# ZechengLi19/CIM

Measured on AMD Instinct MI355X. Metric: images/sec training step (ResNet-50 VOC, ~1k proposals/img) at 1/2/4/8 GPU, higher is better.
Workload: dtype fp32

## Files before the change

cim_amd/csrc/gemm_pair.hip:

```cpp
#include "common.h"
#include <type_traits>
#include "../../include/cim_hip.h"

namespace {

using f32x16 = __attribute__((ext_vector_type(16))) float;
using f16x8 = __attribute__((ext_vector_type(8))) _Float16;
typedef short s16x4 __attribute__((__vector_size__(4 * sizeof(short))));
typedef short s16x8 __attribute__((__vector_size__(8 * sizeof(short))));

#ifndef CIM_PAIR_EXP
#define CIM_PAIR_EXP 0
#endif
static_assert(CIM_PAIR_EXP == 0 || (CIM_PAIR_EXP >= 3 && CIM_PAIR_EXP <= 5), "CIM_PAIR_EXP: 0 (product), 3, 4 or 5");
constexpr bool ABL_NO_LOOP_DMA = CIM_PAIR_EXP == 3 || CIM_PAIR_EXP == 5;
constexpr bool ABL_NO_LOOP_READS = CIM_PAIR_EXP == 4 || CIM_PAIR_EXP == 5;

constexpr int BM = 256, BN = 256, BK = 32;
constexpr int NW = 8, NT = 64 * NW;
constexpr int WNC = 4;
constexpr int WM = 128, WN = BN / WNC, MI = 4, NI = WN / 32;
constexpr int IPW = 32 / NW;
constexpr int OPER = 256 * BK * 4;
constexpr int SLAB = 2 * OPER;
constexpr int LDS_BYTES = 2 * SLAB;
constexpr int RBM = 128, RBK = 16, RNT = 256, RSTAGES = 5;
constexpr int RSTAGE_A = RBM * RBK * 4, RSTAGE_B = BN * RBK * 4, RSTAGE = RSTAGE_A + RSTAGE_B;
constexpr int RIPA = RSTAGE_A / 1024 / 4, RIPB = RSTAGE_B / 1024 / 4;
constexpr int RLDS_BYTES = RSTAGES * RSTAGE;

enum { L_KC = 0, L_MC = 1 };

struct PairArgs {
    const char* A;
    const char* B;
    float* C;
    const float* bias;
    int M, N, K;
    int lda, ldb, ldc;
    int relu;
    int k_per_split;
    long long c_split_stride;
    int batch;
    long long a_bs, b_bs, c_bs;
    const float* a_scale;
    const float* b_scale;
    unsigned* c_amax;
    int tn, tm, tz;
    int tile0;
};

typedef __attribute__((address_space(3))) char* lds_ptr_t;

__device__ __forceinline__ void glds16x4(const char* sbase, unsigned o0, unsigned o1, unsigned o2, unsigned o3, unsigned lds_dst) {
    unsigned keep;
    asm volatile(
        "s_mov_b32 %0, m0\n\t"
        "s_mov_b32 m0, %6\n\t"
        "s_nop 4\n\t"
        "global_load_lds_dwordx4 %1, %5\n\t"
        "s_addk_i32 m0, 0x400\n\t"
        "s_nop 0\n\t"
        "global_load_lds_dwordx4 %2, %5\n\t"
        "s_addk_i32 m0, 0x400\n\t"
        "s_nop 0\n\t"
        "global_load_lds_dwordx4 %3, %5\n\t"
        "s_addk_i32 m0, 0x400\n\t"
        "s_nop 0\n\t"
        "global_load_lds_dwordx4 %4, %5\n\t"
        "s_mov_b32 m0, %0"
        : "=&s"(keep)
// ... 153 lines not shown
__device__ __forceinline__ unsigned abs_bits(float x) { return __float_as_uint(x) & 0x7fffffffu; }
__device__ __forceinline__ unsigned abs_bits(unsigned x) { return x & 0x7fffffffu; }
template <class V4>
__device__ __forceinline__ unsigned abs_bits_max4(const V4& v) {
    return max(max(abs_bits(v.x), abs_bits(v.y)), max(abs_bits(v.z), abs_bits(v.w)));
}

__device__ __forceinline__ void block_amax_publish(unsigned* word, unsigned v) {
    __shared__ unsigned s_m[4];
    v = wave_max_u32(v);
    if ((threadIdx.x & 63) == 0) s_m[threadIdx.x >> 6] = v;
    __syncthreads();
    if (threadIdx.x == 0) cim::amax_publish(word, max(max(s_m[0], s_m[1]), max(s_m[2], s_m[3])));
}

template <int TBM, int SLABK>
struct PairTile {
    int tile_m, tile_n, m0, n0;
    const char* A;
    const char* B;
    float* C;
    int zsplit, zb;
    int kbeg, nslab;
    __device__ __forceinline__ explicit PairTile(const PairArgs& g) {
        int zidx;
        pair_tile_map(g.M, g.N, g.tn, g.tm, g.tz, (int)blockIdx.x + g.tile0, tile_m, tile_n, zidx);
        m0 = tile_m * TBM;
        n0 = tile_n * BN;
        A = g.A;
        B = g.B;
        C = g.C;
        zsplit = zidx;
        zb = 0;
        if (g.batch > 1) {
            A += (size_t)zidx * g.a_bs * 4;
            B += (size_t)zidx * g.b_bs * 4;
            C += (size_t)zidx * g.c_bs;
            zsplit = 0;
            zb = zidx;
        }
        kbeg = zsplit * g.k_per_split;
        const int kend = min(g.K, kbeg + g.k_per_split);
        nslab = (kend - kbeg) / SLABK;
    }
};

__device__ __forceinline__ void pair_acc_init(const PairArgs& g, int ncol0, int lane, f32x16 (&acc)[MI][NI], float (&bvj)[NI]) {
#pragma unroll
    for (int i = 0; i < MI; ++i)
#pragma unroll
        for (int j = 0; j < NI; ++j)
#pragma unroll
            for (int r = 0; r < 16; ++r) acc[i][j][r] = 0.0f;
#pragma unroll
    for (int j = 0; j < NI; ++j) {
        const int n = ncol0 + j * 32 + (lane & 31);
        bvj[j] = (g.bias != nullptr && n < g.N) ? g.bias[n] : 0.0f;
    }
}

template <class Loop>
__device__ __forceinline__ void for_valid_subtiles(int rows, Loop&& loop) {
    switch (__builtin_amdgcn_readfirstlane(min(MI, (rows + 31) / 32))) {
        case 1: loop(std::integral_constant<int, 1>{}); break;
        case 2: loop(std::integral_constant<int, 2>{}); break;
        case 3: loop(std::integral_constant<int, 3>{}); break;
        default: loop(std::integral_constant<int, MI>{}); break;
    }
}

template <int MIV>
struct PairFrags {
    f16x8 ah[MIV > 0 ? MIV : 1], al[MIV > 0 ? MIV : 1], bh[NI], bl[NI];
};

template <int MIV>
__device__ __forceinline__ void mma_cluster(f32x16 (&acc)[MI][NI], const f16x8 (&af)[MIV], const f16x8 (&bf)[NI]) {
#pragma unroll
    for (int i = 0; i < MIV; ++i)
#pragma unroll
        for (int j = 0; j < NI; ++j) acc[i][j] = __builtin_amdgcn_mfma_f32_32x32x16_f16(af[i], bf[j], acc[i][j], 0, 0, 0);
}

template <int NMFMA, int NREAD>
__device__ __forceinline__ void interleave_mfma_reads() {
#pragma unroll
    for (int q = 0; q < NMFMA; ++q) {
        __builtin_amdgcn_sched_group_barrier(0x008, 1, 0);
        if (q < NREAD) __builtin_amdgcn_sched_group_barrier(0x100, 1, 0);
    }
    if constexpr (NREAD > NMFMA) __builtin_amdgcn_sched_group_barrier(0x100, NREAD - NMFMA, 0);
    __builtin_amdgcn_sched_barrier(0);
}

template <int TBM, int SLABK>
__device__ __forceinline__ void pair_epilogue(const PairArgs& g, const PairTile<TBM, SLABK>& T, f32x16 (&acc)[MI][NI], float (&bvj)[NI],
                                              int wm, int wn, int lane) {
    const float inv = 1.0f / (g.a_scale[T.zb] * g.b_scale[T.zb]);
#pragma unroll
    for (int j = 0; j < NI; ++j) asm volatile("" : "+v"(bvj[j]));
    float* C = T.C + (size_t)T.zsplit * g.c_split_stride;
    const int m0 = T.m0, n0 = T.n0;
    const int lk = lane >> 5, l31 = lane & 31;
    unsigned amax = 0;
    const bool relu = g.relu != 0;
    if (m0 + TBM <= g.M && n0 + BN <= g.N) {
#pragma unroll
        for (int j = 0; j < NI; ++j) {
            float* cj = C + (size_t)(m0 + wm * WM + 4 * lk) * g.ldc + n0 + wn * WN + j * 32 + l31;
#pragma unroll
            for (int i = 0; i < MI; ++i) {
#pragma unroll
                for (int r = 0; r < 16; ++r) {
                    float v = acc[i][j][r] * inv + bvj[j];
                    if (relu) v = fmaxf(v, 0.0f);
                    amax = max(amax, abs_bits(v));
                    cj[(size_t)(i * 32 + (r & 3) + 8 * (r >> 2)) * g.ldc] = v;
                }
            }
        }
    } else {
#pragma unroll
        for (int j = 0; j < NI; ++j) {
            const int n = n0 + wn * WN + j * 32 + l31;
            if (n >= g.N) continue;
#pragma unroll
            for (int i = 0; i < MI; ++i) {
#pragma unroll
                for (int r = 0; r < 16; ++r) {
                    const int m = m0 + wm * WM + i * 32 + (r & 3) + 8 * (r >> 2) + 4 * lk;
                    if (m >= g.M) continue;
                    float v = acc[i][j][r] * inv + bvj[j];
                    if (relu) v = fmaxf(v, 0.0f);
                    amax = max(amax, abs_bits(v));
                    C[(size_t)m * g.ldc + n] = v;
                }
            }
        }
    }
    if (g.c_amax != nullptr && g.c_split_stride == 0) {
        amax = wave_max_u32(amax);
        if (lane == 0) cim::amax_publish(g.c_amax, amax);
    }
}

template <int AL, int BL, bool ONEP>
__global__ __launch_bounds__(NT, NW / 4) void gemm_pair_kernel(const PairArgs g) {
    extern __shared__ __attribute__((aligned(16))) char smem[];
    const int tid = threadIdx.x;
    const int wave = __builtin_amdgcn_readfirstlane(tid >> 6), lane = tid & 63;
    const int wm = wave / WNC, wn = wave % WNC;
    const PairTile<BM, BK> T(g);
    const int nslab = T.nslab;

    using StageA = typename StageSel<AL, BM, IPW>::type;
    using StageB = typename StageSel<BL, BN, IPW>::type;
    StageA sa;
    StageB sb;
    sa.init(T.m0, g.M, g.lda, wave, lane);
    sb.init(T.n0, g.N, g.ldb, wave, lane);
    const char* ak = T.A + (AL == L_KC ? (size_t)T.kbeg * 4 : (size_t)T.kbeg * g.lda * 4);
    const char* bk = T.B + (BL == L_KC ? (size_t)T.kbeg * 4 : (size_t)T.kbeg * g.ldb * 4);
    const size_t a_adv = StageA::k_step_bytes(g.lda), b_adv = StageB::k_step_bytes(g.ldb);

    typename FragSel<AL, MI, BM>::type fa;
    typename FragSel<BL, NI, BN>::type fb;
    fa.init(wm * WM, lane);
    fb.init(wn * WN, lane);

    f32x16 acc[MI][NI];
    float bvj[NI];
    pair_acc_init(g, T.n0 + wn * WN, lane, acc, bvj);

    auto issue_slab = [&](const char* buf, auto with_a) __attribute__((always_inline)) {
        if constexpr (decltype(with_a)::value) sa.issue(ak, buf, wave);
        sb.issue(bk, buf + OPER, wave);
        ak += a_adv;
        bk += b_adv;
    };
    auto prologue = [&](auto with_a) __attribute__((always_inline)) {
        issue_slab(smem, with_a);
        asm volatile("s_waitcnt vmcnt(0)" ::: "memory");
        __syncthreads();
        if (nslab > 1) issue_slab(smem + SLAB, with_a);
    };
    auto slab_loop = [&](auto miv_c) {
        constexpr int MIV = decltype(miv_c)::value;
        constexpr std::bool_constant<(MIV > 0 || AL == L_MC)> with_a{};
        PairFrags<MIV> f0, f1;
        auto read = [&](PairFrags<MIV>& f, const char* buf, int ks, auto in_loop) __attribute__((always_inline)) {
            if constexpr (MIV == 0) {
            } else if constexpr (ABL_NO_LOOP_READS && decltype(in_loop)::value) {
                asm volatile("" : "+v"(f.ah[0]), "+v"(f.al[0]), "+v"(f.bh[0]), "+v"(f.bl[0]));
            } else {
#pragma unroll
// ... 50 lines not shown
template <bool ONEP>
__global__ __launch_bounds__(RNT, 2) void gemm_pair_ring_kernel(const PairArgs g) {
    extern __shared__ __attribute__((aligned(16))) char smem[];
    const int tid = threadIdx.x;
    const int wave = __builtin_amdgcn_readfirstlane(tid >> 6), lane = tid & 63;
    const int wn = wave;
    const PairTile<RBM, RBK> T(g);
    const int nslab = T.nslab;

    const char* ak = T.A + (size_t)T.kbeg * g.lda * 4;
    const char* bk = T.B + (size_t)T.kbeg * g.ldb * 4;
    const size_t a_adv = (size_t)RBK * g.lda * 4, b_adv = (size_t)RBK * g.ldb * 4;
    StageMC<RBM, RIPA, RBK> sa;
    StageMC<BN, RIPB, RBK> sb;
    sa.init(T.m0, g.M, g.lda, wave, lane);
    sb.init(T.n0, g.N, g.ldb, wave, lane);
    FragMC<MI, RBM> fa;
    FragMC<NI, BN> fb;
    fa.init(0, lane);
    fb.init(wn * WN, lane);

    f32x16 acc[MI][NI];
    float bvj[NI];
    pair_acc_init(g, T.n0 + wn * WN, lane, acc, bvj);

    int left = nslab - 1;
    auto advance = [&]() __attribute__((always_inline)) {
        const bool more = left > 0;
        ak += more ? a_adv : 0;
        bk += more ? b_adv : 0;
        left -= more ? 1 : 0;
    };
#pragma unroll
    for (int q = 0; q < RSTAGES - 1; ++q) {
        sa.issue(ak, smem + q * RSTAGE, wave);
        sb.issue(bk, smem + q * RSTAGE + RSTAGE_A, wave);
        advance();
    }
    asm volatile("s_waitcnt vmcnt(18)" ::: "memory");
    __syncthreads();

    auto main_loop = [&](auto miv_c) {
        constexpr int MIV = decltype(miv_c)::value;
        PairFrags<MIV> f0, f1;
        auto read_b = [&](PairFrags<MIV>& f, const char* buf) __attribute__((always_inline)) {
#pragma unroll
            for (int j = 0; j < NI; ++j) {
// ... 33 lines not shown
                read_a(nf.ah, nxt, 0);
                mma_cluster(acc, f.ah, f.bh);
                interleave_mfma_reads<MIV * NI, 2 * MIV>();
                sb.issue_pair(bk, wbuf + RSTAGE_A, wave, 1);
            }
            advance();
            wb = wb == RSTAGES - 1 ? 0 : wb + 1;
            rb = rb == RSTAGES - 1 ? 0 : rb + 1;
        };
        read_b(f0, smem);
        if constexpr (!ONEP) read_a(f0.al, smem, 1);
        read_a(f0.ah, smem, 0);
        for (int t = 0; t < nslab; t += 2) {
            step(f0, f1);
            step(f1, f0);
        }
    };
    for_valid_subtiles(g.M - T.m0, main_loop);
    asm volatile("s_waitcnt vmcnt(0)" ::: "memory");
    pair_epilogue(g, T, acc, bvj, 0, wn, lane);
}

__global__ __launch_bounds__(256) void pair_splitk_reduce_kernel(const float* __restrict__ ws, float* __restrict__ C,
                                                                 const float* __restrict__ bias, int M, int N, int ldc,
                                                                 int splits, long long stride, int relu,
                                                                 unsigned* __restrict__ c_amax) {
    const long long total = (long long)M * N;
    unsigned am = 0;
    for (long long i = ((long long)blockIdx.x * 256 + threadIdx.x) * 4; i < total; i += (long long)gridDim.x * 1024) {
        const int m = (int)(i / N), n = (int)(i % N);
        float4 s = *reinterpret_cast<const float4*>(ws + i);
        for (int k0 = 1; k0 < splits; k0 += 4) {
            float4 v[4];
#pragma unroll
            for (int j = 0; j < 4; ++j)
                v[j] = k0 + j < splits ? *reinterpret_cast<const float4*>(ws + (long long)(k0 + j) * stride + i) : make_float4(0.f, 0.f, 0.f, 0.f);
#pragma unroll
            for (int j = 0; j < 4; ++j)
                if (k0 + j < splits) { s.x += v[j].x; s.y += v[j].y; s.z += v[j].z; s.w += v[j].w; }
        }
        if (bias) {
            const float4 b = *reinterpret_cast<const float4*>(bias + n);
            s.x += b.x; s.y += b.y; s.z += b.z; s.w += b.w;
        }
        if (relu) {
            s.x = fmaxf(s.x, 0.f); s.y = fmaxf(s.y, 0.f); s.z = fmaxf(s.z, 0.f); s.w = fmaxf(s.w, 0.f);
        }
        *reinterpret_cast<float4*>(C + (size_t)m * ldc + n) = s;
        am = max(am, abs_bits_max4(s));
    }
    if (c_amax != nullptr) block_amax_publish(c_amax, am);
}

using cim::pair_split2;
using cim::pair_scale_of;

__global__ __launch_bounds__(256) void pair_masked_stats_kernel(const float* __restrict__ dy, const float* __restrict__ y, int rows,
                                                                int cols, float* __restrict__ part, unsigned* __restrict__ amax) {
    __shared__ float4 red[16][16];
// ... 58 lines not shown
            a = make_float4(ya.x > 0.f ? a.x : 0.f, ya.y > 0.f ? a.y : 0.f, ya.z > 0.f ? a.z : 0.f, ya.w > 0.f ? a.w : 0.f);
            b = make_float4(yb.x > 0.f ? b.x : 0.f, yb.y > 0.f ? b.y : 0.f, yb.z > 0.f ? b.z : 0.f, yb.w > 0.f ? b.w : 0.f);
        }
        pair_split2(a.x * s, a.y * s, h.x, l.x);
        pair_split2(a.z * s, a.w * s, h.y, l.y);
        pair_split2(b.x * s, b.y * s, h.z, l.z);
        pair_split2(b.z * s, b.w * s, h.w, l.w);
    }
    char* dst = P + ((size_t)z * p_bs + (size_t)r * ldp + c * 8) * 4;
    *reinterpret_cast<uint4*>(dst) = h;
    *reinterpret_cast<uint4*>(dst + 16) = l;
}

__global__ __launch_bounds__(256) void pair_amax_kernel(const float* __restrict__ X, long long n4, int tail, unsigned* __restrict__ out) {
    unsigned m = 0;
    if (blockIdx.x == 0 && (int)threadIdx.x < tail) m = abs_bits(X[n4 * 4 + threadIdx.x]);
    for (long long i = (long long)blockIdx.x * 256 + threadIdx.x; i < n4; i += (long long)gridDim.x * 256) {
        const uint4 v = *reinterpret_cast<const uint4*>(X + i * 4);
        m = max(m, abs_bits_max4(v));
    }
    block_amax_publish(out, m);
}

template <int AL, int BL, bool RING>
int launch_pair(PairArgs g, int splits, float* workspace, hipStream_t st, int max_workgroups, int products) {
    static_assert(!RING || (AL == L_MC && BL == L_MC), "the ring kernel is the weight gradients' layout only");
    constexpr int TBM = RING ? RBM : BM, LDSB = RING ? RLDS_BYTES : LDS_BYTES, THREADS = RING ? RNT : NT;
    const int tm = (g.M + TBM - 1) / TBM, tn = (g.N + BN - 1) / BN;
    void (*kern)(const PairArgs);
    if constexpr (RING) kern = products == 1 ? gemm_pair_ring_kernel<true> : gemm_pair_ring_kernel<false>;
    else kern = products == 1 ? gemm_pair_kernel<AL, BL, true> : gemm_pair_kernel<AL, BL, false>;
    hipError_t e = hipFuncSetAttribute(reinterpret_cast<const void*>(kern), hipFuncAttributeMaxDynamicSharedMemorySize, LDSB);
    if (e != hipSuccess) return (int)e;
    const int slabs = g.K / BK;
    if (splits < 1) splits = 1;
    if (splits > slabs) splits = slabs;
    g.k_per_split = ((slabs + splits - 1) / splits) * BK;
    splits = (g.K + g.k_per_split - 1) / g.k_per_split;
    float* out = g.C;
    const float* bias = g.bias;
    const int relu = g.relu, ldc = g.ldc;
    if (splits > 1) {
        if (g.batch > 1) return -1;
        g.C = workspace;
        g.ldc = g.N;
        g.c_split_stride = (long long)g.M * g.N;
        g.bias = nullptr;
        g.relu = 0;
    } else {
        g.c_split_stride = 0;
    }
    g.tn = tn; g.tm = tm; g.tz = g.batch > 1 ? g.batch : splits;
    const long long total = (long long)tn * tm * g.tz;
    if (total >= (1ll << 31)) return -2;
    const long long chunk = max_workgroups > 0 ? max_workgroups : total;
    for (long long t0 = 0; t0 < total; t0 += chunk) {
        g.tile0 = (int)t0;
        hipLaunchKernelGGL(kern, dim3((unsigned)(total - t0 < chunk ? total - t0 : chunk)), dim3(THREADS), LDSB, st, g);
    }
    if (splits > 1) {
        const long long quads = ((long long)g.M * g.N + 3) / 4;
        const long long rwgs = (quads + 255) / 256;
        hipLaunchKernelGGL(pair_splitk_reduce_kernel, dim3((unsigned)(rwgs < 1024 ? rwgs : 1024)), dim3(256), 0, st, workspace,
                           out, bias, g.M, g.N, ldc, splits, g.c_split_stride, relu, g.c_amax);
    }
    return 0;
}

int dispatch_pair(const PairArgs& g, int a_mcontig, int b_kcontig, int splits, float* workspace, hipStream_t st, int max_workgroups,
                  int products, int form) {
    if (form == 1) {
        if (a_mcontig && !b_kcontig) return launch_pair<L_MC, L_MC, true>(g, splits, workspace, st, max_workgroups, products);
        return -3;
    }
    if (!a_mcontig && !b_kcontig) return launch_pair<L_KC, L_MC, false>(g, splits, workspace, st, max_workgroups, products);
    if (!a_mcontig && b_kcontig) return launch_pair<L_KC, L_KC, false>(g, splits, workspace, st, max_workgroups, products);
    if (a_mcontig && !b_kcontig) return launch_pair<L_MC, L_MC, false>(g, splits, workspace, st, max_workgroups, products);
    return launch_pair<L_MC, L_KC, false>(g, splits, workspace, st, max_workgroups, products);
}

}

static PairArgs pair_args(const void* A, const void* B, float* C, int M, int N, int K, int lda, int ldb, int ldc, const float* a_scale,
                          const float* b_scale) {
    PairArgs g{};
    g.A = (const char*)A;
    g.B = (const char*)B;
    g.C = C;
    g.M = M;
    g.N = N;
    g.K = K;
    g.lda = lda;
    g.ldb = ldb;
    g.ldc = ldc;
    g.batch = 1;
    g.a_scale = a_scale;
    g.b_scale = b_scale;
    return g;
}

static bool pair_dims_ok(int M, int N, int K, int lda, int ldb, int ldc, int a_mcontig, int b_kcontig) {
// ... 4 lines not shown
    const long long ext_a = (long long)(a_mcontig ? K : M) * lda * 4, ext_b = (long long)(b_kcontig ? N : K) * ldb * 4;
    if (ext_a >= (1ll << 32) || ext_b >= (1ll << 32)) return false;
    return true;
}

extern "C" int cim_gemm_pair_splits(int M, int N, int K) {
    const double CUS = 256.0;
    const double tiles = (double)((M + 255) / 256) * ((N + BN - 1) / BN);
    const int slabs = K / BK;
    const double flops = 2.0 * M * (double)N * K;
    int best = 1;
    double best_t = 1e30;
    for (int s = 1; s <= 16; ++s) {
        if (s > 1 && slabs / s < 8) break;
        const double units = tiles * s;
        const double rounds = (double)(long long)((units + CUS - 1) / CUS);
        const double eff = units / (rounds * CUS);
        const double t = flops / (420e12 * eff) + (s > 1 ? (2.0 * s + 1.0) * M * (double)N * 4.0 / 4e12 : 0.0);
        if (t < best_t) { best_t = t; best = s; }
    }
    return best;
}

extern "C" int cim_gemm_pair(const void* A, const void* B, float* C, const float* bias, int M, int N, int K, int lda,
                             int ldb, int ldc, int a_mcontig, int b_kcontig, int relu, int splits, float* workspace,
                             const float* a_scale, const float* b_scale, uint32_t* c_amax, int max_workgroups, int products,
                             int form, void* stream) {
    CIM_CHECK_ARG(A && B && C && a_scale && b_scale && max_workgroups >= 0 && (products == 3 || products == 1));
    CIM_CHECK_ARG(form == 0 || (form == 1 && a_mcontig && !b_kcontig));
    CIM_CHECK_ARG(pair_dims_ok(M, N, K, lda, ldb, ldc, a_mcontig, b_kcontig));
    CIM_CHECK_ARG(splits <= 1 || workspace != nullptr);
    PairArgs g = pair_args(A, B, C, M, N, K, lda, ldb, ldc, a_scale, b_scale);
    g.bias = bias;
    g.relu = relu;
    g.c_amax = c_amax;
    int rc = dispatch_pair(g, a_mcontig, b_kcontig, splits, workspace, cim::as_stream(stream), max_workgroups, products, form);
    if (rc) { cim::set_error("cim_gemm_pair: launch setup failed (%d)", rc); return rc; }
    CIM_CHECK_LAUNCH();
    return 0;
}

extern "C" int cim_gemm_pair_batched(const void* A, const void* B, float* C, int M, int N, int K, int lda, int ldb,
                                     int ldc, int a_mcontig, int b_kcontig, int batch, long long a_bs, long long b_bs,
                                     long long c_bs, const float* a_scale, const float* b_scale, int max_workgroups, int products,
                                     int form, void* stream) {
    CIM_CHECK_ARG(A && B && C && a_scale && b_scale && batch > 0 && batch <= 65535 && max_workgroups >= 0 && (products == 3 || products == 1));
    CIM_CHECK_ARG(form == 0 || (form == 1 && a_mcontig && !b_kcontig));
    CIM_CHECK_ARG(pair_dims_ok(M, N, K, lda, ldb, ldc, a_mcontig, b_kcontig));
    CIM_CHECK_ARG(a_bs % 8 == 0 && b_bs % 8 == 0 && c_bs % 4 == 0);
    PairArgs g = pair_args(A, B, C, M, N, K, lda, ldb, ldc, a_scale, b_scale);
    g.batch = batch;
    g.a_bs = a_bs;
    g.b_bs = b_bs;
    g.c_bs = c_bs;
    int rc = dispatch_pair(g, a_mcontig, b_kcontig, 1, nullptr, cim::as_stream(stream), max_workgroups, products, form);
    if (rc) { cim::set_error("cim_gemm_pair_batched: launch setup failed (%d)", rc); return rc; }
    CIM_CHECK_LAUNCH();
    return 0;
}

extern "C" int cim_pair_scales(const uint32_t* amax, int n_amax, const float* factor, float* scale, int n, int reduce_all, void* stream) {
    CIM_CHECK_ARG(amax && scale && n > 0 && n_amax > 0);
    hipLaunchKernelGGL(pair_scales_kernel, dim3((n + 255) / 256), dim3(256), 0, cim::as_stream(stream), amax, n_amax, factor, scale, n,
                       reduce_all);
    CIM_CHECK_LAUNCH();
    return 0;
}

extern "C" int cim_pair_split(const float* X, void* P, int rows, int rows_pad, int cols, int ld, int ldp, int batch,
                              long long x_bs, long long p_bs, const float* scale, const float* relu_y, void* stream) {
    CIM_CHECK_ARG(X && P && scale && rows > 0 && rows_pad >= rows && cols > 0 && batch > 0 && batch <= 65535);
    CIM_CHECK_ARG(cols % 8 == 0 && ld % 4 == 0 && ld >= cols && ldp % 8 == 0 && ldp >= cols && x_bs % 4 == 0 && p_bs % 8 == 0);
    const long long chunks = (long long)rows_pad * (cols / 8);
    hipLaunchKernelGGL(pair_split_kernel, dim3((unsigned)((chunks + 255) / 256), batch), dim3(256), 0, cim::as_stream(stream), X,
                       (char*)P, rows, rows_pad, cols, ld, ldp, x_bs, p_bs, scale, relu_y);
    CIM_CHECK_LAUNCH();
    return 0;
}
// ... 18 lines not shown
```

cim_amd/ops/pair.py:

```python
import torch

from .. import _lib


def pad32(n):
    return (n + 31) & ~31


class Pair:
    __slots__ = ("buf", "rows", "cols", "batch", "scale")

    def __init__(self, buf, rows, cols, batch, scale):
        self.buf, self.rows, self.cols, self.batch, self.scale = buf, rows, cols, batch, scale

    @property
    def rows_pad(self):
        return self.buf.shape[-2]

    @property
    def ld(self):
        return self.buf.shape[-1]

    @property
    def bs(self):
# ... 59 lines not shown
    tail = (tn - main_tn) * tm
    if main_tn == 0 or tail > 64:
        return None
    s = 1
    while s * 2 * tail <= 256 and k // (s * 2 * 32) >= 8 and s < 16:
        s *= 2
    return (main_tn * 256, s) if s > 1 else None


def tail_entries(m, n, k, batch):
    t = ((m + 255) // 256) * ((n + 255) // 256)
    rem = (batch * t) % 256
    if batch * t <= 256 or rem == 0 or rem > 64 or rem % t:
        return None
    s = 1
    while s * 2 * t <= 256 and k // (s * 2 * 32) >= 8 and s < 16:
        s *= 2
    return (rem // t, s) if s > 1 else None


PRODUCTS = 3


def gemm(a, b, m, n, k, a_mcontig=False, b_kcontig=False, bias=None, relu=False, out=None, c_amax=None, balance=False, limit=0,
         products=None, form=0):
    dev = a.buf.device
    products = PRODUCTS if products is None else products
    if a.batch > 1:
        c = out if out is not None else torch.empty((a.batch, m, n), dtype=torch.float32, device=dev)
        tail = tail_entries(m, n, k, a.batch) if balance else None
        main = a.batch - (tail[0] if tail else 0)
        _lib.call("cim_gemm_pair_batched", a.buf.data_ptr(), b.buf.data_ptr(), c.data_ptr(), m, n, k, a.ld, b.ld, n,
                  int(a_mcontig), int(b_kcontig), main, a.bs, b.bs, m * n, a.scale.data_ptr(), b.scale.data_ptr(),
                  limit, products, form, _lib.stream_ptr())
        if tail:
            ws = torch.empty(tail[1] * m * n, dtype=torch.float32, device=dev)
            for z in range(main, a.batch):
                _lib.call("cim_gemm_pair", a.buf.data_ptr() + 4 * z * a.bs, b.buf.data_ptr() + 4 * z * b.bs, c.data_ptr() + 4 * z * m * n,
                          None, m, n, k, a.ld, b.ld, n, int(a_mcontig), int(b_kcontig), 0, tail[1], ws.data_ptr(),
                          a.scale.data_ptr() + 4 * z, b.scale.data_ptr() + 4 * z, None, limit, products, form, _lib.stream_ptr())
        return c
    c = out if out is not None else torch.empty((m, n), dtype=torch.float32, device=dev)
    splits = _lib.call("cim_gemm_pair_splits", m, n, k)
    tail = tail_columns(m, n, k) if (balance and splits == 1) else None
    if tail is not None:
        n_main, s = tail
        n_tail = n - n_main
        ws = torch.empty(s * m * n_tail, dtype=torch.float32, device=dev)
        b_off = (n_main * b.ld if b_kcontig else n_main) * 4
        for (cols, col0, boff, sp, w) in ((n_main, 0, 0, 1, None), (n_tail, n_main, b_off, s, ws)):
            _lib.call("cim_gemm_pair", a.buf.data_ptr(), b.buf.data_ptr() + boff, c.data_ptr() + 4 * col0,
                      (bias.data_ptr() + 4 * col0) if bias is not None else None, m, cols, k, a.ld, b.ld, n,
                      int(a_mcontig), int(b_kcontig), int(relu), sp, _lib.ptr(w), a.scale.data_ptr(), b.scale.data_ptr(),
                      _lib.ptr(c_amax), limit, products, form, _lib.stream_ptr())
        return c
    ws = torch.empty(splits * m * n, dtype=torch.float32, device=dev) if splits > 1 else None
    _lib.call("cim_gemm_pair", a.buf.data_ptr(), b.buf.data_ptr(), c.data_ptr(), _lib.ptr(bias), m, n, k, a.ld, b.ld, n,
              int(a_mcontig), int(b_kcontig), int(relu), splits, _lib.ptr(ws), a.scale.data_ptr(), b.scale.data_ptr(),
              _lib.ptr(c_amax), limit, products, form, _lib.stream_ptr())
    return c
```

include/cim_hip.h:

```cpp
#ifndef CIM_HIP_H
#define CIM_HIP_H

#include <stdint.h>

#ifdef __cplusplus
extern "C" {
#endif

const char* cim_last_error(void);
int cim_abi_version(void);

int cim_roi_align_fwd(const float* feat, const float* rois, float* out,
                      int B, int C, int H, int W, int K, int P,
                      float spatial_scale, int sampling_ratio, int aligned, void* stream);

long long cim_roi_align_bwd_workspace(int K, int P, int H, int W);
int cim_roi_align_bwd(const float* grad_out, const float* rois, float* grad_in,
                      int B, int C, int H, int W, int K, int P,
                      float spatial_scale, int sampling_ratio, int aligned, float* workspace, void* stream);

int cim_roi_align_fwd_ws(const float* feat, const float* rois, float* out,
                         int B, int C, int H, int W, int K, int P,
                         float spatial_scale, int sampling_ratio, int aligned, float* workspace, void* stream);
int cim_roi_align_maskcat_fwd_ws(const float* feat, const float* rois, const float* masks, float* cat,
// ... 236 lines not shown
int cim_conv3x3_wt_multi(const cim_wt_desc* descs, int n, void* stream);

long long cim_conv7x7_dw_workspace(int B, int cin, int cout, int H, int W, int stride);
int cim_conv7x7_dw_splits(int B, int cin, int cout, int H, int W, int stride);
int cim_conv7x7_dw_f32(const float* dconv, const float* x, float* dw, int B, int cin, int cout, int H, int W, int stride,
                       float* workspace, void* stream);

int cim_bn_act_fwd(const float* x, const float* res, const float* gamma, const float* beta, const float* mean,
                   const float* var, float eps, float* y, int N, int C, int HW, int relu, void* stream);
int cim_bn_act_bwd_chunks(int N, int C, int HW);
int cim_bn_act_bwd(const float* dy, const float* y, const float* x, const float* gamma, const float* mean,
                   const float* var, float eps, float* dx, float* dres, float* dgamma, float* dbeta,
                   int N, int C, int HW, int relu, void* stream);

int cim_gemm_pair_splits(int M, int N, int K);
int cim_gemm_pair(const void* A, const void* B, float* C, const float* bias, int M, int N, int K,
                  int lda, int ldb, int ldc, int a_mcontig, int b_kcontig, int relu, int splits, float* workspace,
                  const float* a_scale, const float* b_scale, uint32_t* c_amax, int max_workgroups, int products, int form,
                  void* stream);
int cim_gemm_pair_batched(const void* A, const void* B, float* C, int M, int N, int K,
                          int lda, int ldb, int ldc, int a_mcontig, int b_kcontig,
                          int batch, long long a_bs, long long b_bs, long long c_bs,
                          const float* a_scale, const float* b_scale, int max_workgroups, int products, int form, void* stream);
int cim_pair_scales(const uint32_t* amax, int n_amax, const float* factor, float* scale, int n, int reduce_all, void* stream);
int cim_pair_split(const float* X, void* P, int rows, int rows_pad, int cols, int ld, int ldp, int batch,
                   long long x_bs, long long p_bs, const float* scale, const float* relu_y, void* stream);
int cim_pair_amax(const float* X, long long n, uint32_t* amax, void* stream);
int cim_pair_masked_stats(const float* dy, const float* y, int rows, int cols, float* part, uint32_t* amax, void* stream);

int cim_wino7_pair_scales(const uint32_t* amax, int n_amax, const uint32_t* amax_mul, int kind, float* scale, void* stream);
int cim_wino7_input_pair(const float* x, void* V, const float* scale, int R, int Rs, int C, void* stream);
int cim_wino7_filter_pair(const float* W, void* U, const float* scale, int Cout, int Cin, void* stream);
int cim_wino7_dy_pair(const float* dy, void* D, const float* scale, int R, int Rs, int C, int adjoint, void* stream);
int cim_wino7_flatten_bwd_dy_pair(const float* dX, const float* relu_y, void* E, const float* scale_e, void* D, const float* scale_d,
                                  float* bias_partial, int R, int Rs, int C, void* stream);
int cim_wino7_output_amax(const float* M, const float* bias, float* y, int R, int C, int relu, uint32_t* y_amax, void* stream);
int cim_flatten_chw_pair(const float* src, void* dst, const float* scale, int R, int Rs, int PP, int C, void* stream);
int cim_flatten_chw_bwd_bias(const float* src, const float* relu_y, float* dst, float* bias_partial, int R, int PP, int C,
                             void* stream);


int cim_wino_wgrad_output(const float* dU, float* dW, int Cout, int Cin, int tile, void* stream);
int cim_wino_dx_adjoint_output(const float* M, float* dx, int R, int P, int C, int tile, void* stream);
int cim_wino7_dx_maskfold(const float* M, const float* masks, float* dbox, int R, int Cb, void* stream);

#define CIM_PCL_MAX_CLUSTERS 256
// ... 80 lines not shown
```

Before: 75.76.

## Split-K ragged row tiles separately using a cost-model planner for pair GEMM

Lets the pair GEMM use different split-K factors for full row tiles and the ragged final row tile in a single launch, with a reduce kernel that handles both workspace regions. Adds a host-side planner that models tile cost and list-schedules work units over workgroup slots to choose the splits and the tail balancing, cached per shape in Python. The aim is less load imbalance and tail idle time on the compute units when M is not a multiple of the tile height. In exchange it adds workspace traffic and a reduce pass, and the per-shape choices depend on hand-tuned cost constants.

```diff
diff --git a/cim_amd/csrc/gemm_pair.hip b/cim_amd/csrc/gemm_pair.hip
--- a/cim_amd/csrc/gemm_pair.hip
+++ b/cim_amd/csrc/gemm_pair.hip
@@ -1,5 +1,8 @@
 #include "common.h"
+#include <functional>
+#include <queue>
 #include <type_traits>
+#include <vector>
 #include "../../include/cim_hip.h"
 
 namespace {
@@ -39,14 +42,18 @@
     int M, N, K;
     int lda, ldb, ldc;
     int relu;
-    int k_per_split;
-    long long c_split_stride;
     int batch;
     long long a_bs, b_bs, c_bs;
     const float* a_scale;
     const float* b_scale;
     unsigned* c_amax;
-    int tn, tm, tz;
+    int tn, tm_full, tm_rag, z_full, z_rag;
+    int units_full;
+    int kps_full, kps_rag;
+    float* C_rag;
+    int ldc_rag;
+    long long stride_full, stride_rag;
+    int final_full, final_rag;
     int tile0;
 };
 
@@ -246,14 +253,23 @@
     float* C;
     int zsplit, zb;
     int kbeg, nslab;
+    int ldc;
+    long long split_stride;
+    bool final;
     __device__ __forceinline__ explicit PairTile(const PairArgs& g) {
+        const int vb = (int)blockIdx.x + g.tile0;
+        const bool rag = vb >= g.units_full;
         int zidx;
-        pair_tile_map(g.M, g.N, g.tn, g.tm, g.tz, (int)blockIdx.x + g.tile0, tile_m, tile_n, zidx);
+        pair_tile_map(g.M, g.N, g.tn, rag ? g.tm_rag : g.tm_full, rag ? g.z_rag : g.z_full, rag ? vb - g.units_full : vb, tile_m, tile_n, zidx);
+        if (rag) tile_m += g.tm_full;
         m0 = tile_m * TBM;
         n0 = tile_n * BN;
         A = g.A;
         B = g.B;
-        C = g.C;
+        C = rag ? g.C_rag : g.C;
+        ldc = rag ? g.ldc_rag : g.ldc;
+        split_stride = rag ? g.stride_rag : g.stride_full;
+        final = (rag ? g.final_rag : g.final_full) != 0;
         zsplit = zidx;
         zb = 0;
         if (g.batch > 1) {
@@ -263,13 +279,14 @@
             zsplit = 0;
             zb = zidx;
         }
-        kbeg = zsplit * g.k_per_split;
-        const int kend = min(g.K, kbeg + g.k_per_split);
+        const int kps = rag ? g.kps_rag : g.kps_full;
+        kbeg = zsplit * kps;
+        const int kend = min(g.K, kbeg + kps);
         nslab = (kend - kbeg) / SLABK;
     }
 };
 
-__device__ __forceinline__ void pair_acc_init(const PairArgs& g, int ncol0, int lane, f32x16 (&acc)[MI][NI], float (&bvj)[NI]) {
+__device__ __forceinline__ void pair_acc_init(const PairArgs& g, bool final, int ncol0, int lane, f32x16 (&acc)[MI][NI], float (&bvj)[NI]) {
 #pragma unroll
     for (int i = 0; i < MI; ++i)
 #pragma unroll
@@ -279,7 +296,7 @@
 #pragma unroll
     for (int j = 0; j < NI; ++j) {
         const int n = ncol0 + j * 32 + (lane & 31);
-        bvj[j] = (g.bias != nullptr && n < g.N) ? g.bias[n] : 0.0f;
+        bvj[j] = (final && g.bias != nullptr && n < g.N) ? g.bias[n] : 0.0f;
     }
 }
 
@@ -323,15 +340,15 @@
     const float inv = 1.0f / (g.a_scale[T.zb] * g.b_scale[T.zb]);
 #pragma unroll
     for (int j = 0; j < NI; ++j) asm volatile("" : "+v"(bvj[j]));
-    float* C = T.C + (size_t)T.zsplit * g.c_split_stride;
-    const int m0 = T.m0, n0 = T.n0;
+    float* C = T.C + (size_t)T.zsplit * T.split_stride;
+    const int m0 = T.m0, n0 = T.n0, ldc = T.ldc;
     const int lk = lane >> 5, l31 = lane & 31;
     unsigned amax = 0;
-    const bool relu = g.relu != 0;
+    const bool relu = T.final && g.relu != 0;
     if (m0 + TBM <= g.M && n0 + BN <= g.N) {
 #pragma unroll
         for (int j = 0; j < NI; ++j) {
-            float* cj = C + (size_t)(m0 + wm * WM + 4 * lk) * g.ldc + n0 + wn * WN + j * 32 + l31;
+            float* cj = C + (size_t)(m0 + wm * WM + 4 * lk) * ldc + n0 + wn * WN + j * 32 + l31;
 #pragma unroll
             for (int i = 0; i < MI; ++i) {
 #pragma unroll
@@ -339,7 +356,7 @@
                     float v = acc[i][j][r] * inv + bvj[j];
                     if (relu) v = fmaxf(v, 0.0f);
                     amax = max(amax, abs_bits(v));
-                    cj[(size_t)(i * 32 + (r & 3) + 8 * (r >> 2)) * g.ldc] = v;
+                    cj[(size_t)(i * 32 + (r & 3) + 8 * (r >> 2)) * ldc] = v;
                 }
             }
         }
@@ -357,12 +374,12 @@
                     float v = acc[i][j][r] * inv + bvj[j];
                     if (relu) v = fmaxf(v, 0.0f);
                     amax = max(amax, abs_bits(v));
-                    C[(size_t)m * g.ldc + n] = v;
+                    C[(size_t)m * ldc + n] = v;
                 }
             }
         }
     }
-    if (g.c_amax != nullptr && g.c_split_stride == 0) {
+    if (g.c_amax != nullptr && T.final) {
         amax = wave_max_u32(amax);
         if (lane == 0) cim::amax_publish(g.c_amax, amax);
     }
@@ -394,7 +411,7 @@
 
     f32x16 acc[MI][NI];
     float bvj[NI];
-    pair_acc_init(g, T.n0 + wn * WN, lane, acc, bvj);
+    pair_acc_init(g, T.final, T.n0 + wn * WN, lane, acc, bvj);
 
     auto issue_slab = [&](const char* buf, auto with_a) __attribute__((always_inline)) {
         if constexpr (decltype(with_a)::value) sa.issue(ak, buf, wave);
@@ -491,7 +508,7 @@
 
     f32x16 acc[MI][NI];
     float bvj[NI];
-    pair_acc_init(g, T.n0 + wn * WN, lane, acc, bvj);
+    pair_acc_init(g, T.final, T.n0 + wn * WN, lane, acc, bvj);
 
     int left = nslab - 1;
     auto advance = [&]() __attribute__((always_inline)) {
@@ -571,19 +588,23 @@
 }
 
 __global__ __launch_bounds__(256) void pair_splitk_reduce_kernel(const float* __restrict__ ws, float* __restrict__ C,
-                                                                 const float* __restrict__ bias, int M, int N, int ldc,
-                                                                 int splits, long long stride, int relu,
-                                                                 unsigned* __restrict__ c_amax) {
-    const long long total = (long long)M * N;
+                                                                 const float* __restrict__ bias, int M, int N, int ldc, int row_beg,
+                                                                 int row_end, int m_rag, int s_full, int s_rag, long long off_rag,
+                                                                 int relu, unsigned* __restrict__ c_amax) {
+    const long long first = (long long)row_beg * N, total = (long long)row_end * N;
     unsigned am = 0;
-    for (long long i = ((long long)blockIdx.x * 256 + threadIdx.x) * 4; i < total; i += (long long)gridDim.x * 1024) {
+    for (long long i = first + ((long long)blockIdx.x * 256 + threadIdx.x) * 4; i < total; i += (long long)gridDim.x * 1024) {
         const int m = (int)(i / N), n = (int)(i % N);
-        float4 s = *reinterpret_cast<const float4*>(ws + i);
+        const bool rag = m >= m_rag;
+        const int splits = rag ? s_rag : s_full;
+        const long long stride = (long long)(rag ? M - m_rag : m_rag) * N;
+        const float* p = rag ? ws + off_rag + (i - (long long)m_rag * N) : ws + i;
+        float4 s = *reinterpret_cast<const float4*>(p);
         for (int k0 = 1; k0 < splits; k0 += 4) {
             float4 v[4];
 #pragma unroll
             for (int j = 0; j < 4; ++j)
-                v[j] = k0 + j < splits ? *reinterpret_cast<const float4*>(ws + (long long)(k0 + j) * stride + i) : make_float4(0.f, 0.f, 0.f, 0.f);
+                v[j] = k0 + j < splits ? *reinterpret_cast<const float4*>(p + (long long)(k0 + j) * stride) : make_float4(0.f, 0.f, 0.f, 0.f);
 #pragma unroll
             for (int j = 0; j < 4; ++j)
                 if (k0 + j < splits) { s.x += v[j].x; s.y += v[j].y; s.z += v[j].z; s.w += v[j].w; }
@@ -688,8 +709,31 @@
     block_amax_publish(out, m);
 }
 
+struct PairCut {
+    int s_full, s_rag;
+    bool by_class;
+};
+static void pair_cut_k(int K, int& splits, int& kps) {
+    const int slabs = K / BK;
+    splits = splits < 1 ? 1 : (splits > slabs ? slabs : splits);
+    kps = ((slabs + splits - 1) / splits) * BK;
+    splits = (K + kps - 1) / kps;
+}
+static long long pair_cut_workspace(int M, int N, int K, PairCut cut, int* m_rag_out = nullptr, long long* off_rag_out = nullptr,
+                                    int* kps_out = nullptr) {
+    int kps[2];
+    pair_cut_k(K, cut.s_full, kps[0]);
+    pair_cut_k(K, cut.s_rag, kps[1]);
+    const int m_rag = (cut.by_class && M % BM) ? M / BM * BM : M;
+    const long long off_rag = cut.s_full > 1 ? (long long)cut.s_full * m_rag * N : 0;
+    if (m_rag_out) *m_rag_out = m_rag;
+    if (off_rag_out) *off_rag_out = off_rag;
+    if (kps_out) { kps_out[0] = kps[0]; kps_out[1] = kps[1]; }
+    return off_rag + ((m_rag < M && cut.s_rag > 1) ? (long long)cut.s_rag * (M - m_rag) * N : 0);
+}
+
 template <int AL, int BL, bool RING>
-int launch_pair(PairArgs g, int splits, float* workspace, hipStream_t st, int max_workgroups, int products) {
+int launch_pair(PairArgs g, PairCut cut, float* workspace, hipStream_t st, int max_workgroups, int products) {
     static_assert(!RING || (AL == L_MC && BL == L_MC), "the ring kernel is the weight gradients' layout only");
     constexpr int TBM = RING ? RBM : BM, LDSB = RING ? RLDS_BYTES : LDS_BYTES, THREADS = RING ? RNT : NT;
     const int tm = (g.M + TBM - 1) / TBM, tn = (g.N + BN - 1) / BN;
@@ -698,51 +742,72 @@
     else kern = products == 1 ? gemm_pair_kernel<AL, BL, true> : gemm_pair_kernel<AL, BL, false>;
     hipError_t e = hipFuncSetAttribute(reinterpret_cast<const void*>(kern), hipFuncAttributeMaxDynamicSharedMemorySize, LDSB);
     if (e != hipSuccess) return (int)e;
-    const int slabs = g.K / BK;
-    if (splits < 1) splits = 1;
-    if (splits > slabs) splits = slabs;
-    g.k_per_split = ((slabs + splits - 1) / splits) * BK;
-    splits = (g.K + g.k_per_split - 1) / g.k_per_split;
+    int kps[2], m_rag;
+    long long off_rag;
+    pair_cut_k(g.K, cut.s_full, kps[0]);
+    pair_cut_k(g.K, cut.s_rag, kps[1]);
+    if (cut.s_full == cut.s_rag) cut.by_class = false;
+    pair_cut_workspace(g.M, g.N, g.K, cut, &m_rag, &off_rag, kps);
+    const bool has_rag = m_rag < g.M;
+    if (!has_rag) cut.s_rag = 1;
+    if (m_rag == 0) cut.s_full = 1;
+    const bool split_full = cut.s_full > 1, split_rag = has_rag && cut.s_rag > 1;
+    if ((split_full || split_rag) && (g.batch > 1 || workspace == nullptr)) return -1;
     float* out = g.C;
-    const float* bias = g.bias;
-    const int relu = g.relu, ldc = g.ldc;
-    if (splits > 1) {
-        if (g.batch > 1) return -1;
+    const int ldc = g.ldc;
+    g.tn = tn;
+    g.tm_full = m_rag / TBM;
+    if (!has_rag) g.tm_full = tm;
+    g.tm_rag = tm - g.tm_full;
+    g.z_full = g.batch > 1 ? g.batch : cut.s_full;
+    g.z_rag = cut.s_rag;
+    g.kps_full = kps[0];
+    g.kps_rag = kps[1];
+    g.C_rag = out;
+    g.ldc_rag = ldc;
+    g.stride_full = g.stride_rag = 0;
+    g.final_full = g.final_rag = 1;
+    if (split_full) {
         g.C = workspace;
         g.ldc = g.N;
-        g.c_split_stride = (long long)g.M * g.N;
-        g.bias = nullptr;
-        g.relu = 0;
-    } else {
-        g.c_split_stride = 0;
-    }
-    g.tn = tn; g.tm = tm; g.tz = g.batch > 1 ? g.batch : splits;
-    const long long total = (long long)tn * tm * g.tz;
+        g.stride_full = (long long)m_rag * g.N;
+        g.final_full = 0;
+    }
+    if (split_rag) {
+        g.C_rag = reinterpret_cast<float*>(reinterpret_cast<uintptr_t>(workspace + off_rag) - (uintptr_t)m_rag * g.N * sizeof(float));
+        g.ldc_rag = g.N;
+        g.stride_rag = (long long)(g.M - m_rag) * g.N;
+        g.final_rag = 0;
+    }
+    const long long units_full = (long long)tn * g.tm_full * g.z_full;
+    const long long total = units_full + (long long)tn * g.tm_rag * g.z_rag;
     if (total >= (1ll << 31)) return -2;
+    g.units_full = (int)units_full;
     const long long chunk = max_workgroups > 0 ? max_workgroups : total;
     for (long long t0 = 0; t0 < total; t0 += chunk) {
         g.tile0 = (int)t0;
         hipLaunchKernelGGL(kern, dim3((unsigned)(total - t0 < chunk ? total - t0 : chunk)), dim3(THREADS), LDSB, st, g);
     }
-    if (splits > 1) {
-        const long long quads = ((long long)g.M * g.N + 3) / 4;
+    if (split_full || split_rag) {
+        const int row_beg = split_full ? 0 : m_rag, row_end = split_rag ? g.M : m_rag;
+        const long long quads = ((long long)(row_end - row_beg) * g.N + 3) / 4;
         const long long rwgs = (quads + 255) / 256;
         hipLaunchKernelGGL(pair_splitk_reduce_kernel, dim3((unsigned)(rwgs < 1024 ? rwgs : 1024)), dim3(256), 0, st, workspace,
-                           out, bias, g.M, g.N, ldc, splits, g.c_split_stride, relu, g.c_amax);
+                           out, g.bias, g.M, g.N, ldc, row_beg, row_end, m_rag, cut.s_full, cut.s_rag, off_rag, g.relu, g.c_amax);
     }
     return 0;
 }
 
-int dispatch_pair(const PairArgs& g, int a_mcontig, int b_kcontig, int splits, float* workspace, hipStream_t st, int max_workgroups,
+int dispatch_pair(const PairArgs& g, int a_mcontig, int b_kcontig, PairCut cut, float* workspace, hipStream_t st, int max_workgroups,
                   int products, int form) {
     if (form == 1) {
-        if (a_mcontig && !b_kcontig) return launch_pair<L_MC, L_MC, true>(g, splits, workspace, st, max_workgroups, products);
+        if (a_mcontig && !b_kcontig) return launch_pair<L_MC, L_MC, true>(g, cut, workspace, st, max_workgroups, products);
         return -3;
     }
-    if (!a_mcontig && !b_kcontig) return launch_pair<L_KC, L_MC, false>(g, splits, workspace, st, max_workgroups, products);
-    if (!a_mcontig && b_kcontig) return launch_pair<L_KC, L_KC, false>(g, splits, workspace, st, max_workgroups, products);
-    if (a_mcontig && !b_kcontig) return launch_pair<L_MC, L_MC, false>(g, splits, workspace, st, max_workgroups, products);
-    return launch_pair<L_MC, L_KC, false>(g, splits, workspace, st, max_workgroups, products);
+    if (!a_mcontig && !b_kcontig) return launch_pair<L_KC, L_MC, false>(g, cut, workspace, st, max_workgroups, products);
+    if (!a_mcontig && b_kcontig) return launch_pair<L_KC, L_KC, false>(g, cut, workspace, st, max_workgroups, products);
+    if (a_mcontig && !b_kcontig) return launch_pair<L_MC, L_MC, false>(g, cut, workspace, st, max_workgroups, products);
+    return launch_pair<L_MC, L_KC, false>(g, cut, workspace, st, max_workgroups, products);
 }
 
 }
@@ -793,6 +858,153 @@
     return best;
 }
 
+constexpr double PLAN_US_SLAB = 2.65, PLAN_RING_RATE = 1.55 / 2.89, PLAN_REDUCE_BPUS = 3.3e6, PLAN_US_REDUCE = 4.0;
+constexpr double PLAN_TILE_COST[8] = {0.53, 0.56, 0.60, 0.62, 0.70, 0.76, 0.93, 1.0}, PLAN_RING_TILE_COST[4] = {0.93, 0.96, 0.96, 1.0};
+constexpr double PLAN_IMBALANCE = 0.35, PLAN_MIN_GAIN = 0.03;
+constexpr int PLAN_SLOTS = 256, PLAN_MIN_SLABS = 8, PLAN_MAX_SPLITS = 16;
+
+static double pair_tile_cost(int rows, int form) {
+    const int v = (rows + 31) / 32;
+    return form == 1 ? PLAN_RING_TILE_COST[(v < 4 ? v : 4) - 1] : PLAN_TILE_COST[(v < 8 ? v : 8) - 1];
+}
+static double pair_unit_us(int rows) { return 2.0 + 14.0 * rows / 256.0; }
+
+namespace {
+struct PairShape {
+    int M, N, K, form;
+    int tile_rows() const { return form == 1 ? RBM : BM; }
+    int tm() const { return (M + tile_rows() - 1) / tile_rows(); }
+    int tn() const { return (N + BN - 1) / BN; }
+    int rag_rows() const { return M % BM; }
+    int tm_full() const { return (M - rag_rows()) / tile_rows(); }
+};
+struct UnitGroup {
+    long long n;
+    double us;
+};
+
+double pair_list_schedule(const UnitGroup* groups, int ngroups) {
+    std::priority_queue<double, std::vector<double>, std::greater<double>> free_at;
+    for (int i = 0; i < PLAN_SLOTS; ++i) free_at.push(0.0);
+    double end = 0.0;
+    for (int g = 0; g < ngroups; ++g) {
+        long long n = groups[g].n;
+        if (n >= 2 * PLAN_SLOTS) {
+            const long long rounds = n / PLAN_SLOTS - 1;
+            std::vector<double> t;
+            for (; !free_at.empty(); free_at.pop()) t.push_back(free_at.top() + rounds * groups[g].us);
+            for (double x : t) free_at.push(x);
+            n -= rounds * PLAN_SLOTS;
+        }
+        for (long long u = 0; u < n; ++u) {
+            const double t = free_at.top() + groups[g].us;
+            free_at.pop();
+            free_at.push(t);
+            if (t > end) end = t;
+        }
+    }
+    return end;
+}
+
+double pair_cut_time(const PairShape& p, int& s_full, int& s_rag, long long* units_out) {
+    int kf, kr;
+    pair_cut_k(p.K, s_full, kf);
+    pair_cut_k(p.K, s_rag, kr);
+    const double us_slab = p.form == 1 ? PLAN_US_SLAB * PLAN_RING_RATE : PLAN_US_SLAB;
+    const int tmf = p.tm_full(), rag = p.rag_rows();
+    if (!rag) s_rag = s_full;
+    if (!tmf) s_full = s_rag;
+    const int rag_a = rag > p.tile_rows() ? p.tile_rows() : rag, rag_b = rag - rag_a;
+    const UnitGroup groups[3] = {{(long long)p.tn() * tmf * s_full, pair_unit_us(p.tile_rows()) + kf / 32.0 * us_slab},
+                                 {rag_a ? p.tn() * s_rag : 0, pair_unit_us(rag_a) + kr / 32.0 * us_slab * pair_tile_cost(rag_a, p.form)},
+                                 {rag_b ? p.tn() * s_rag : 0, pair_unit_us(rag_b) + kr / 32.0 * us_slab * pair_tile_cost(rag_b, p.form)}};
+    if (units_out) *units_out = groups[0].n + groups[1].n + groups[2].n;
+    double work = 0;
+    for (const UnitGroup& g : groups) work += g.n * g.us / PLAN_SLOTS;
+    const double list = pair_list_schedule(groups, 3);
+    double t = work + PLAN_IMBALANCE * (list > work ? list - work : 0.0);
+    double bytes = 0;
+    if (s_full > 1) bytes += (s_full + 1.0) * (p.M - rag) * p.N * 4.0;
+    if (s_rag > 1) bytes += (s_rag + 1.0) * rag * p.N * 4.0;
+    if (bytes > 0) t += PLAN_US_REDUCE + bytes / PLAN_REDUCE_BPUS;
+    return t;
+}
+
+void pair_best_cut(const PairShape& p, int& best_f, int& best_r, long long* units_out) {
+    const int min_k = PLAN_MIN_SLABS * (p.form == 1 ? RBK : BK);
+    best_f = best_r = cim_gemm_pair_splits(p.M, p.N, p.K);
+    double best = pair_cut_time(p, best_f, best_r, units_out) * (1.0 - PLAN_MIN_GAIN);
+    if (!p.rag_rows() || !p.tm_full()) return;
+    for (int sf = 1; sf <= PLAN_MAX_SPLITS; ++sf) {
+        if (sf > 1 && p.K / sf < min_k) break;
+        for (int sr = 1; sr <= PLAN_MAX_SPLITS; ++sr) {
+            if (sr > 1 && p.K / sr < min_k) break;
+            int f = sf, r = sr;
+            long long units;
+            const double t = pair_cut_time(p, f, r, &units);
+            if (t < best) {
+                best = t;
+                best_f = f;
+                best_r = r;
+                if (units_out) *units_out = units;
+            }
+        }
+    }
+}
+}
+
+extern "C" int cim_gemm_pair_plan(int M, int N, int K, int batch, int form, int balance, long long* plan) {
+    CIM_CHECK_ARG(M > 0 && N > 0 && K > 0 && K % 32 == 0 && batch > 0 && (form == 0 || form == 1) && plan != nullptr);
+    const PairShape p{M, N, K, form};
+    for (int i = 0; i < CIM_PAIR_PLAN_WORDS; ++i) plan[i] = 0;
+    plan[0] = plan[1] = plan[4] = plan[5] = 1;
+    const long long tiles = (long long)p.tm() * p.tn();
+    long long units = tiles * batch, ws = 0;
+    int sf = 1, sr = 1;
+    if (batch == 1) {
+        pair_best_cut(p, sf, sr, &units);
+        ws = pair_cut_workspace(M, N, K, PairCut{sf, sr, true});
+    }
+    plan[0] = sf;
+    plan[1] = sr;
+    if (balance && form == 0 && sf == 1 && sr == 1 && tiles * batch > PLAN_SLOTS) {
+        const long long rem = (tiles * batch) % PLAN_SLOTS;
+        if (batch > 1) {
+            if (rem != 0 && rem <= 64 && rem % tiles == 0) {
+                int s = 1;
+                while ((long long)s * 2 * tiles <= PLAN_SLOTS && K / (s * 2 * 32) >= PLAN_MIN_SLABS && s < PLAN_MAX_SPLITS) s *= 2;
+                if (s > 1) {
+                    plan[2] = 2; plan[3] = rem / tiles; plan[4] = plan[5] = s;
+                    ws = pair_cut_workspace(M, N, K, PairCut{s, s, true});
+                    units = tiles * (batch - plan[3]);
+                }
+            }
+        } else if (rem != 0 && N % BN == 0) {
+            int main_tn = p.tn();
+            while (main_tn > 0 && ((long long)main_tn * p.tm()) % PLAN_SLOTS) --main_tn;
+            const long long tail = (long long)(p.tn() - main_tn) * p.tm();
+            if (main_tn > 0 && tail <= 64) {
+                int s = 1;
+                while ((long long)s * 2 * tail <= PLAN_SLOTS && K / (s * 2 * 32) >= PLAN_MIN_SLABS && s < PLAN_MAX_SPLITS) s *= 2;
+                if (s > 1) {
+                    plan[2] = 1; plan[3] = N - main_tn * BN; plan[4] = plan[5] = s;
+                    ws = pair_cut_workspace(M, (int)plan[3], K, PairCut{s, s, true});
+                    units = (long long)main_tn * p.tm();
+                }
+            }
+        }
+    }
+    plan[6] = ws;
+    plan[7] = units;
+    plan[8] = (units + PLAN_SLOTS - 1) / PLAN_SLOTS;
+    return 0;
+}
+
+extern "C" long long cim_gemm_pair_cut_workspace(int M, int N, int K, int s_full, int s_rag) {
+    if (M <= 0 || N <= 0 || K <= 0 || K % 32 != 0) return -1;
+    return pair_cut_workspace(M, N, K, PairCut{s_full, s_rag, true});
+}
+
 extern "C" int cim_gemm_pair(const void* A, const void* B, float* C, const float* bias, int M, int N, int K, int lda,
                              int ldb, int ldc, int a_mcontig, int b_kcontig, int relu, int splits, float* workspace,
                              const float* a_scale, const float* b_scale, uint32_t* c_amax, int max_workgroups, int products,
@@ -805,8 +1017,27 @@
     g.bias = bias;
     g.relu = relu;
     g.c_amax = c_amax;
-    int rc = dispatch_pair(g, a_mcontig, b_kcontig, splits, workspace, cim::as_stream(stream), max_workgroups, products, form);
+    int rc = dispatch_pair(g, a_mcontig, b_kcontig, PairCut{splits, splits, false}, workspace, cim::as_stream(stream), max_workgroups, products, form);
     if (rc) { cim::set_error("cim_gemm_pair: launch setup failed (%d)", rc); return rc; }
+    CIM_CHECK_LAUNCH();
+    return 0;
+}
+
+extern "C" int cim_gemm_pair_cut(const void* A, const void* B, float* C, const float* bias, int M, int N, int K, int lda,
+                                 int ldb, int ldc, int a_mcontig, int b_kcontig, int relu, int s_full, int s_rag, float* workspace,
+                                 const float* a_scale, const float* b_scale, uint32_t* c_amax, int max_workgroups, int products,
+                                 int form, void* stream) {
+    CIM_CHECK_ARG(A && B && C && a_scale && b_scale && max_workgroups >= 0 && (products == 3 || products == 1));
+    CIM_CHECK_ARG(form == 0 || (form == 1 && a_mcontig && !b_kcontig));
+    CIM_CHECK_ARG(pair_dims_ok(M, N, K, lda, ldb, ldc, a_mcontig, b_kcontig));
+    CIM_CHECK_ARG(s_full >= 1 && s_rag >= 1);
+    CIM_CHECK_ARG(workspace != nullptr || pair_cut_workspace(M, N, K, PairCut{s_full, s_rag, true}) == 0);
+    PairArgs g = pair_args(A, B, C, M, N, K, lda, ldb, ldc, a_scale, b_scale);
+    g.bias = bias;
+    g.relu = relu;
+    g.c_amax = c_amax;
+    int rc = dispatch_pair(g, a_mcontig, b_kcontig, PairCut{s_full, s_rag, true}, workspace, cim::as_stream(stream), max_workgroups, products, form);
+    if (rc) { cim::set_error("cim_gemm_pair_cut: launch setup failed (%d)", rc); return rc; }
     CIM_CHECK_LAUNCH();
     return 0;
 }
@@ -824,7 +1055,7 @@
     g.a_bs = a_bs;
     g.b_bs = b_bs;
     g.c_bs = c_bs;
-    int rc = dispatch_pair(g, a_mcontig, b_kcontig, 1, nullptr, cim::as_stream(stream), max_workgroups, products, form);
+    int rc = dispatch_pair(g, a_mcontig, b_kcontig, PairCut{1, 1, false}, nullptr, cim::as_stream(stream), max_workgroups, products, form);
     if (rc) { cim::set_error("cim_gemm_pair_batched: launch setup failed (%d)", rc); return rc; }
     CIM_CHECK_LAUNCH();
     return 0;
diff --git a/cim_amd/ops/pair.py b/cim_amd/ops/pair.py
--- a/cim_amd/ops/pair.py
+++ b/cim_amd/ops/pair.py
@@ -1,3 +1,6 @@
+import ctypes
+import functools
+
 import torch
 
 from .. import _lib
@@ -105,40 +108,47 @@
 PRODUCTS = 3
 
 
+def plan(m, n, k, batch=1, form=0, balance=False):
+    return _plan(int(m), int(n), int(k), int(batch), int(form), bool(balance))
+
+
+@functools.lru_cache(maxsize=None)
+def _plan(m, n, k, batch, form, balance):
+    words = (ctypes.c_longlong * _lib.CONSTANTS["CIM_PAIR_PLAN_WORDS"])()
+    _lib.call("cim_gemm_pair_plan", m, n, k, batch, form, int(balance), ctypes.addressof(words))
+    w = list(words)
+    tail = None if w[2] == 0 else (("columns", "entries")[w[2] - 1], w[3], w[4], w[5])
+    return dict(s_full=w[0], s_rag=w[1], tail=tail, ws=w[6], units=w[7], rounds=w[8])
+
+
 def gemm(a, b, m, n, k, a_mcontig=False, b_kcontig=False, bias=None, relu=False, out=None, c_amax=None, balance=False, limit=0,
          products=None, form=0):
     dev = a.buf.device
     products = PRODUCTS if products is None else products
+    pl = plan(m, n, k, a.batch, 0, balance)
+    ws = torch.empty(pl["ws"], dtype=torch.float32, device=dev) if pl["ws"] else None
+    tail = pl["tail"]
+    st = _lib.stream_ptr()
+
+    def cut(z, cols, col0, s_full, s_rag):
+        b_off = (col0 * b.ld if b_kcontig else col0) * 4
+        _lib.call("cim_gemm_pair_cut", a.buf.data_ptr() + 4 * z * a.bs, b.buf.data_ptr() + 4 * z * b.bs + b_off,
+                  c.data_ptr() + 4 * (z * m * n + col0), (bias.data_ptr() + 4 * col0) if bias is not None else None, m, cols, k,
+                  a.ld, b.ld, n, int(a_mcontig), int(b_kcontig), int(relu), s_full, s_rag, _lib.ptr(ws),
+                  a.scale.data_ptr() + 4 * z, b.scale.data_ptr() + 4 * z, _lib.ptr(c_amax), limit, products, form, st)
+
     if a.batch > 1:
         c = out if out is not None else torch.empty((a.batch, m, n), dtype=torch.float32, device=dev)
-        tail = tail_entries(m, n, k, a.batch) if balance else None
-        main = a.batch - (tail[0] if tail else 0)
+        main = a.batch - (tail[1] if tail else 0)
         _lib.call("cim_gemm_pair_batched", a.buf.data_ptr(), b.buf.data_ptr(), c.data_ptr(), m, n, k, a.ld, b.ld, n,
                   int(a_mcontig), int(b_kcontig), main, a.bs, b.bs, m * n, a.scale.data_ptr(), b.scale.data_ptr(),
-                  limit, products, form, _lib.stream_ptr())
-        if tail:
-            ws = torch.empty(tail[1] * m * n, dtype=torch.float32, device=dev)
-            for z in range(main, a.batch):
-                _lib.call("cim_gemm_pair", a.buf.data_ptr() + 4 * z * a.bs, b.buf.data_ptr() + 4 * z * b.bs, c.data_ptr() + 4 * z * m * n,
-                          None, m, n, k, a.ld, b.ld, n, int(a_mcontig), int(b_kcontig), 0, tail[1], ws.data_ptr(),
-                          a.scale.data_ptr() + 4 * z, b.scale.data_ptr() + 4 * z, None, limit, products, form, _lib.stream_ptr())
+                  limit, products, form, st)
+        for z in range(main, a.batch):
+            cut(z, n, 0, tail[2], tail[3])
         return c
     c = out if out is not None else torch.empty((m, n), dtype=torch.float32, device=dev)
-    splits = _lib.call("cim_gemm_pair_splits", m, n, k)
-    tail = tail_columns(m, n, k) if (balance and splits == 1) else None
-    if tail is not None:
-        n_main, s = tail
-        n_tail = n - n_main
-        ws = torch.empty(s * m * n_tail, dtype=torch.float32, device=dev)
-        b_off = (n_main * b.ld if b_kcontig else n_main) * 4
-        for (cols, col0, boff, sp, w) in ((n_main, 0, 0, 1, None), (n_tail, n_main, b_off, s, ws)):
-            _lib.call("cim_gemm_pair", a.buf.data_ptr(), b.buf.data_ptr() + boff, c.data_ptr() + 4 * col0,
-                      (bias.data_ptr() + 4 * col0) if bias is not None else None, m, cols, k, a.ld, b.ld, n,
-                      int(a_mcontig), int(b_kcontig), int(relu), sp, _lib.ptr(w), a.scale.data_ptr(), b.scale.data_ptr(),
-                      _lib.ptr(c_amax), limit, products, form, _lib.stream_ptr())
-        return c
-    ws = torch.empty(splits * m * n, dtype=torch.float32, device=dev) if splits > 1 else None
-    _lib.call("cim_gemm_pair", a.buf.data_ptr(), b.buf.data_ptr(), c.data_ptr(), _lib.ptr(bias), m, n, k, a.ld, b.ld, n,
-              int(a_mcontig), int(b_kcontig), int(relu), splits, _lib.ptr(ws), a.scale.data_ptr(), b.scale.data_ptr(),
-              _lib.ptr(c_amax), limit, products, form, _lib.stream_ptr())
+    n_main = n - (tail[1] if tail else 0)
+    cut(0, n_main, 0, pl["s_full"], pl["s_rag"])
+    if tail:
+        cut(0, n - n_main, n_main, tail[2], tail[3])
     return c
diff --git a/include/cim_hip.h b/include/cim_hip.h
--- a/include/cim_hip.h
+++ b/include/cim_hip.h
@@ -282,6 +282,13 @@
                           int lda, int ldb, int ldc, int a_mcontig, int b_kcontig,
                           int batch, long long a_bs, long long b_bs, long long c_bs,
                           const float* a_scale, const float* b_scale, int max_workgroups, int products, int form, void* stream);
+#define CIM_PAIR_PLAN_WORDS 9
+int cim_gemm_pair_plan(int M, int N, int K, int batch, int form, int balance, long long* plan);
+long long cim_gemm_pair_cut_workspace(int M, int N, int K, int s_full, int s_rag);
+int cim_gemm_pair_cut(const void* A, const void* B, float* C, const float* bias, int M, int N, int K,
+                      int lda, int ldb, int ldc, int a_mcontig, int b_kcontig, int relu, int s_full, int s_rag, float* workspace,
+                      const float* a_scale, const float* b_scale, uint32_t* c_amax, int max_workgroups, int products, int form,
+                      void* stream);
 int cim_pair_scales(const uint32_t* amax, int n_amax, const float* factor, float* scale, int n, int reduce_all, void* stream);
 int cim_pair_split(const float* X, void* P, int rows, int rows_pad, int cols, int ld, int ldp, int batch,
                    long long x_bs, long long p_bs, const float* scale, const float* relu_y, void* stream);
```

Result: no change. 75.51, median of 2 (-0.3%).
